# crabml/crabml

Hardware: NVIDIA H100
Metric: decode_tokens_per_s (higher is better)
Workload: dtype int8

## Files before the change

### crabml_b200/csrc/common.cuh

```cuda
#pragma once

#include <cuda_fp16.h>
#include <cuda_runtime.h>
#include <stdint.h>

#include <atomic>
#include <map>
#include <mutex>
#include <set>
#include <string>
#include <unordered_map>
#include <vector>

#include "../../include/crabml_cuda.h"

#define QK_K 256

#define CC_D_STRIDE(nb) ((((nb) + 7) / 8) * 8)
#define CC_HAS_PADDED_D(t) ((t) == CC_Q8_0 || (t) == CC_Q4_0)
#define CC_MAX_PLANES 4
#define CC_N_SLOTS 16
#define CC_HISTORY_CAP 65536

struct cc_device;
// ... 195 lines not shown
struct AttnArgs {
    const float *q, *k, *v;
    void *kcache, *vcache;
    float* out;
    void* act_scratch;
    const int64_t* dyn;
    const float* rope_tab;
    int n_heads, n_kv, hd, rope_dim, max_len, kv_f16;
    int64_t seq_stride;
    float scale;
};
struct DeqPlanes { const uint8_t* p[CC_MAX_PLANES]; int64_t cols; };
enum { MK_NORMQ = 0, MK_MATVEC = 1, MK_ATTN = 2, MK_ROWS = 3, MK_REDUCE = 4, MK_GATHER = 5, MK_ARGMAX = 6, MK_SAMPLE = 7 };
struct MkPhase {
    int type, wtype, write_back, next_matvec;
    int xgpu, red_n, spare1, spare; float* red_dst; const float* red_res;
    float* x; float* orig; const float* norm_w; float eps; int n; ActQ8_0 act;
    int act_type, spare2;
    StreamArgs mv;
    AttnArgs at;
    unsigned long long dyn_off, rope_off;
    DeqPlanes planes; int src_dtype, dst_dtype, n_rows, pad; long long cols; void* dst;
    const long long* rows_dev;
    long long* slot_dev; long long* hist_dev;
};
size_t cc_mega_smem_for_phase(const MkPhase& ph);
const CommDev* cc_comm_dev(cc_device* dev);
bool cc_comm_is_nccl(cc_device* dev);
int cc_comm_world(cc_device* dev);
void cc_comm_destroy(cc_device* dev);
int cc_launch_all_reduce(cc_device* dev, float* x, int64_t n, const float* residual);
int cc_launch_all_gather(cc_device* dev, const float* src, int64_t n, float* dst);
extern "C" CC_API int cc_test_mega_barrier_floor(cc_device* dev, int n, float* us_per_phase);
int cc_launch_mega(cc_device* dev, const MkPhase* phases_dev, int n_phases, const uint8_t* dyn_dev, unsigned* bar_dev, size_t smem_work, size_t smem_wstage,
                   unsigned long long* prof, bool sample);
bool cc_mega_test_stall();
bool cc_mega_ring_phase_ok(const MkPhase& ph);
int cc_mega_ring_at_ch(const MkPhase& ph);
size_t cc_mega_ring_smem_for_phase(const MkPhase& ph);
// ... 104 lines not shown
```

### crabml_b200/csrc/lazy.cu

```cuda
#include <math.h>
#include <stdlib.h>
#include <string.h>

#include <chrono>
#include <functional>

#include "sample_dev.cuh"

enum LKind { L_COPY_ROWS, L_DUP, L_RMS_NORM, L_MUL, L_ADD, L_SCALE, L_MATVEC, L_ROPE, L_CONCAT, L_CONTIGUOUS, L_BMM, L_SOFTMAX, L_SILU, L_GELU, L_ALLREDUCE, L_ALLGATHER, L_ARGMAX, L_SAMPLE };

struct LView { cc_buf* buf = nullptr; int ndim = 0; int64_t shape[CC_MAX_DIMS] = {0, 0, 0, 0}, strides[CC_MAX_DIMS] = {0, 0, 0, 0}; };

struct LOp {
    int kind;
    LView a, b;
    cc_buf* out = nullptr;
    float f = 0.0f;
    int64_t i0 = 0, i1 = 0, i2 = 0;
    std::vector<int64_t> rows;
    bool done = false;
};

struct GraphEntry { cudaGraphExec_t exec = nullptr; size_t dyn_bytes = 0; uint64_t launches = 0; MkPhase* phases_dev = nullptr;
                    std::vector<uint64_t> sig; uint64_t last_use = 0; int mega_variant = 0; };
// ... 38 lines not shown
static void graph_entry_free(GraphEntry& ge) {
    if (ge.exec) cudaGraphExecDestroy(ge.exec);
    if (ge.phases_dev) cudaFree(ge.phases_dev);
    ge.exec = nullptr; ge.phases_dev = nullptr;
}
static void graph_cache_clear(LazyState* lz) {
    for (auto& kv : lz->cache) graph_entry_free(kv.second);
    lz->cache.clear();
}

LazyState* cc_lazy_create(cc_device* dev) {
    LazyState* lz = new LazyState();
    for (int i = 0; i < LZ_DYN_SLOTS; i++)
        if (cudaMallocHost(&lz->dyn_host[i], lz->dyn_cap) != cudaSuccess || cudaEventCreateWithFlags(&lz->dyn_ev[i], cudaEventDisableTiming) != cudaSuccess) { delete lz; return nullptr; }
    if (cudaMalloc(&lz->dyn_dev, lz->dyn_cap) != cudaSuccess) { delete lz; return nullptr; }
    if (getenv("CRABML_MEGA_PROF")) cudaMalloc(&lz->prof_dev, 8 * 8 * 4097);
    if (cudaMalloc(&lz->bar_dev, 4096) != cudaSuccess || cudaMemset(lz->bar_dev, 0, 4096) != cudaSuccess) { delete lz; return nullptr; }
    return lz;
}
void cc_lazy_destroy(cc_device* dev) {
    LazyState* lz = dev->lz;
    if (!lz) return;
    for (auto& op : lz->q) { if (op.a.buf) cc_tensor_release(op.a.buf); if (op.b.buf) cc_tensor_release(op.b.buf); if (op.out) cc_tensor_release(op.out); }
    for (auto& kv : lz->cache) graph_entry_free(kv.second);
    lz->cache.clear();
    if (lz->bar_dev) cudaFree(lz->bar_dev);
    for (int i = 0; i < LZ_DYN_SLOTS; i++) { if (lz->dyn_host[i]) cudaFreeHost(lz->dyn_host[i]); if (lz->dyn_ev[i]) cudaEventDestroy(lz->dyn_ev[i]); }
    if (lz->dyn_dev) cudaFree(lz->dyn_dev);
    for (int i = 0; i < 2; i++) if (lz->act[i]) cudaFree(lz->act[i]);
    delete lz;
    dev->lz = nullptr;
// ... 47 lines not shown
    cc_device* dev;
    LazyState* lz;
    std::vector<LOp>& q;
    Plan& P;
    size_t rope_off = (size_t)-1; int64_t rope_pos = -1; int rope_hd = 0, rope_dim = 0;

    bool is(size_t i, int kind) const { return i < q.size() && !q[i].done && q[i].kind == kind; }
    std::unordered_map<cc_buf*, size_t> last_use;
    void index_uses() {
        last_use.reserve(q.size() * 2);
        for (size_t j = 0; j < q.size(); j++) {
            if (q[j].a.buf) last_use[q[j].a.buf] = j;
            if (q[j].b.buf) last_use[q[j].b.buf] = j;
            if (q[j].out) last_use[q[j].out] = j;
        }
    }
    bool dead_after(cc_buf* b, size_t from) const {
        auto lu = last_use.find(b);
        if (lu != last_use.end() && lu->second >= from) return false;
        auto it = lz->qrefs.find(b);
        int held = it == lz->qrefs.end() ? 0 : it->second;
        return b->refs.load() == held;
    }
    static bool same_dense_1xN(const LView& v, int64_t n) { return vcontig(v) && vlen(v) == n; }

    bool covered_by_phase = false;
    void fallback(size_t i) {
        if (!covered_by_phase) P.mega_ok = false;
        LOp op = q[i];
        cc_device* d = dev;
// ... 74 lines not shown
        if (rn.a.ndim > 2 || (rn.a.ndim == 2 && rn.a.shape[0] != 1) || !vcontig(rn.a) || n % 32) return 0;
        if (vlen(mu.b) != n || mu.b.buf->dtype != CC_F32 || !vcontig(mu.b)) return 0;
        if (n > 65536) return 0;
        float* x = (float*)rn.a.buf->plane[0];
        float* og = orig ? (float*)orig->base : nullptr;
        const float* w = (const float*)mu.b.buf->plane[0];
        float eps = rn.f;
        void* act = lz->act[act_sel];
        cc_device* d = dev;
        size_t end = j + 2;
        while (is(end, L_MATVEC) && q[end].b.buf == rn.a.buf && cc_stream_supported(q[end].a.buf->dtype, q[end].a.shape[1]) &&
               vlen(q[end].b) == q[end].a.shape[1] && vcontig(q[end].b)) end++;
        const bool write_back = !dead_after(rn.a.buf, end);
        P.S(0x2001); P.SP(x); P.SP(og); P.SP(w); P.SP(act); P.S((uint64_t)n); uint32_t eb; memcpy(&eb, &eps, 4); P.S(eb); P.S(write_back);
        P.steps.push_back([=](uint8_t*) { return cc_launch_normq(d, x, og, w, eps, n, act, write_back); });
        { MkPhase ph = {}; ph.type = MK_NORMQ; ph.write_back = write_back; ph.x = x; ph.orig = og; ph.norm_w = w; ph.eps = eps; ph.n = (int)n; ph.act = cc_act_q8_0(act, n); P.phases.push_back(ph); }
        *xbuf = rn.a.buf;
        size_t used = (j + 2) - i;
        for (size_t t = i; t < i + used; t++) q[t].done = true;
        return used;
    }

    size_t try_stream(size_t i, cc_buf* xbuf, int act_sel) {
        if (!is(i, L_MATVEC)) return 0;
        const LOp& m0 = q[i];
        const int wt = m0.a.buf->dtype;
        const int64_t k = m0.a.shape[1];
        if (!cc_stream_supported(wt, k) || m0.b.buf != xbuf || vlen(m0.b) != k || !vcontig(m0.b)) return 0;
        size_t n = 1;
        while (n < 3 && is(i + n, L_MATVEC) && q[i + n].b.buf == xbuf && q[i + n].a.buf->dtype == wt && q[i + n].a.shape[1] == k && vlen(q[i + n].b) == k) n++;
        StreamArgs A = {};
// ... 212 lines not shown
        } else if (n > 1 && is(j + n, L_SILU)) { n = 1; used_mv = 1; }
        if (is(j + used_mv, L_ALLREDUCE) || is(j + used_mv, L_ALLGATHER)) return 0;
        const size_t end = j + used_mv;
        if (norm_w && !dead_after(xb, end)) return 0;
        A.mats.n = (int)n;
        for (size_t t = 0; t < n; t++) {
            const cc_buf* w = q[j + t].a.buf;
            if (w->cols != k) return 0;
            A.mats.qs[t] = w->plane[0]; A.mats.d[t] = (const uint16_t*)w->plane[1]; A.mats.p2[t] = w->plane[2]; A.mats.p3[t] = w->plane[3];
            A.mats.out[t] = (float*)q[j + t].out->base;
            A.mats.m[t] = (int)q[j + t].a.shape[0];
        }
        MkPhase ph = {};
        ph.type = MK_MATVEC; ph.wtype = wt; ph.act_type = CC_Q8_K; ph.mv = A;
        ph.x = (float*)xb->plane[0]; ph.orig = orig ? (float*)orig->base : nullptr; ph.norm_w = norm_w; ph.eps = eps; ph.n = (int)k;
        covered_by_phase = true;
        for (size_t t = i; t < end; t++) fallback(t);
        covered_by_phase = false;
        P.phases.push_back(ph);
        P.mega_generic = true;
        return end - i;
    }

    void merge_prologue(size_t at) {
        const bool tail = at + 3 == P.phases.size() && (P.phases[at + 2].type == MK_REDUCE || P.phases[at + 2].type == MK_GATHER);
        if (at + 2 != P.phases.size() && !tail) return;
        MkPhase& nq = P.phases[at];
        MkPhase& mv = P.phases[at + 1];
        if (nq.type != MK_NORMQ || mv.type != MK_MATVEC || nq.write_back || nq.n != mv.mv.k) return;
        mv.x = nq.x; mv.orig = nq.orig; mv.norm_w = nq.norm_w; mv.eps = nq.eps; mv.n = nq.n;
        P.phases.erase(P.phases.begin() + at);
        if (at >= 1 && P.phases[at - 1].type == MK_REDUCE && P.phases[at - 1].red_dst == P.phases[at].x && P.phases[at - 1].red_n == P.phases[at].n) {
            MkPhase& m2 = P.phases[at];
            m2.red_n = P.phases[at - 1].red_n; m2.red_res = P.phases[at - 1].red_res;
            P.phases.erase(P.phases.begin() + (at - 1));
        }
    }

    void run() {
        index_uses();
        size_t i = 0;
        while (i < q.size()) {
            if (q[i].done) { i++; continue; }
            size_t used;
            cc_buf* xb = nullptr;
// ... 101 lines not shown
            if (use_mega && P.mega_sample) {
                int n_sample = 0;
                for (auto& ph : P.phases) n_sample += ph.type == MK_SAMPLE;
                if (n_sample != 1 || P.phases.back().type != MK_SAMPLE) use_mega = false;
            }
            if (use_mega) {
                bool stream = false, ring_ok = true;
                for (auto& ph : P.phases) {
                    if (ph.type == MK_MATVEC && ph.act_type != CC_Q8_K) stream = true;
                    if (!cc_mega_ring_phase_ok(ph)) ring_ok = false;
                }
                P.mega_ring = stream;
                for (auto& ph : P.phases) {
                    if (P.mega_ring) {
                        P.mega_smem = std::max(P.mega_smem, cc_mega_ring_smem_for_phase(ph));
                        if (ph.type == MK_MATVEC && ph.act_type == CC_Q8_K && ph.x && ph.norm_w) P.mega_wstage = std::max(P.mega_wstage, (size_t)ph.n * 4);
                        if (ph.type == MK_MATVEC && ph.act_type != CC_Q8_K) P.ring_slot = std::max(P.ring_slot, ph.wtype == CC_Q8_0 ? 4352 : 2304);
                        if (ph.type == MK_ATTN) P.ring_at_ch = cc_mega_ring_at_ch(ph);
                    } else {
                        P.mega_smem = std::max(P.mega_smem, cc_mega_smem_for_phase(ph));
                        if (ph.type == MK_MATVEC && ph.x && ph.norm_w) P.mega_wstage = std::max(P.mega_wstage, (size_t)ph.n * 4);
                    }
                }
                if (P.mega_ring) use_mega = ring_ok && cc_mega_ring_fits(P.mega_smem, P.mega_wstage, P.ring_slot, P.mega_generic);
                else use_mega = P.mega_smem + P.mega_wstage + 4096 <= 227 * 1024;
            }
            if (use_mega) {
                int nxt = -1;
                for (int t = (int)P.phases.size() - 1; t >= 0; t--) {
                    P.phases[t].next_matvec = nxt;
                    if (P.phases[t].type == MK_MATVEC) nxt = t;
                }
                if (cudaMalloc(&ge.phases_dev, P.phases.size() * sizeof(MkPhase)) != cudaSuccess ||
                    cudaMemcpy(ge.phases_dev, P.phases.data(), P.phases.size() * sizeof(MkPhase), cudaMemcpyHostToDevice) != cudaSuccess)
                    rc = cc_fail(dev, CC_ERR_CUDA, "lazy: phase table upload failed");
            }
            cudaError_t e = rc ? cudaSuccess : cudaStreamBeginCapture(dev->stream, cudaStreamCaptureModeRelaxed);
            if (!rc && e != cudaSuccess) rc = cc_fail(dev, CC_ERR_CUDA, "lazy: begin capture: %s", cudaGetErrorString(e));
            if (!rc) {
                if (use_mega && lz->prof_dev && P.phases.size() < 4000) { lz->prof_types.clear(); for (auto& ph : P.phases) lz->prof_types.push_back(ph.type * 16 + (ph.type == MK_MATVEC ? ph.mv.mats.n + 4 * ph.mv.epilogue + 1024 * (ph.mv.k >> 10) : 0)); }
                unsigned long long* prof = P.phases.size() < 4000 ? lz->prof_dev : nullptr;
                if (!use_mega) rc = run_steps(lz->dyn_dev);
                else if (P.mega_ring) rc = cc_launch_mega_ring(dev, ge.phases_dev, (int)P.phases.size(), lz->dyn_dev, lz->bar_dev, P.mega_smem, P.mega_wstage, prof, cc_comm_dev(dev),
                                                               P.mega_generic, P.mega_sample, P.ring_slot, P.ring_at_ch);
                else rc = cc_launch_mega(dev, ge.phases_dev, (int)P.phases.size(), lz->dyn_dev, lz->bar_dev, P.mega_smem, P.mega_wstage, prof, P.mega_sample);
                e = cudaStreamEndCapture(dev->stream, &graph);
// ... 39 lines not shown
int cc_check_async_error(cc_device* dev) {
    if (!dev || !dev->err_host) return CC_OK;
    const unsigned code = *(volatile unsigned*)dev->err_host;
    if (!code) return CC_OK;
    *(volatile unsigned*)dev->err_host = 0u;
    if (dev->err_dev) cudaMemset(dev->err_dev, 0, 256);
    if (dev->lz && dev->lz->bar_dev) cudaMemset(dev->lz->bar_dev, 0, 4096);
    return cc_fail(dev, CC_ERR_CUDA, "%s timeout (%s): the grid was not co-resident or a peer GPU stopped responding",
                   code == 3u ? "exchange kernel" : "megakernel barrier", code == 1u ? "grid barrier" : code == 4u ? "weight ring" : "cross-GPU handshake");
}

extern "C" CC_API int cc_lazy_mega_profile(cc_device* dev, unsigned long long* ts, int* types, int cap, int* n_out) {
    if (!dev || !dev->lz || !dev->lz->prof_dev || !ts || !types || !n_out) return CC_ERR_ARG;
    cudaStreamSynchronize(dev->stream);
    int n = (int)dev->lz->prof_types.size();
    if ((n + 1) * 8 > cap) return CC_ERR_ARG;
    if (cudaMemcpy(ts, dev->lz->prof_dev, (size_t)(n + 1) * 8 * 8, cudaMemcpyDeviceToHost) != cudaSuccess) return CC_ERR_CUDA;
    for (int i = 0; i < n; i++) types[i] = dev->lz->prof_types[i];
    *n_out = n;
    return CC_OK;
}

extern "C" CC_API int cc_lazy_mega_variant(cc_device* dev) { return dev && dev->lz ? dev->lz->mega_variant : 0; }

extern "C" CC_API int cc_lazy_stats(cc_device* dev, uint64_t* out4) {
    if (!dev || !dev->lz || !out4) return CC_ERR_ARG;
    out4[0] = dev->lz->flushes; out4[1] = dev->lz->graph_hits; out4[2] = dev->lz->captures; out4[3] = dev->lz->uncached;
    out4[4] = dev->lz->ns_record; out4[5] = dev->lz->ns_fuse; out4[6] = dev->lz->ns_submit; out4[7] = dev->lz->n_ops;
    return CC_OK;
}
```

### crabml_b200/csrc/mega_phases.cuh

```cuda
#pragma once
#include <stdlib.h>
#include <string.h>

#include "common.cuh"
#include "dequant.cuh"
#include "quantize_dev.cuh"
#include "vecdot.cuh"
#include "sample_dev.cuh"

#ifndef MK_SYNC
#error "define MK_SYNC() before including mega_phases.cuh"
#endif

#define MK_THREADS 512
#define MK_WARPS 16
#define MK_CTAS_PER_SM 1
#define MK_SEG 4
#define MK_XSTAGE_ROWS 512

__device__ __forceinline__ unsigned ld_acquire_u32(const unsigned* p) {
    unsigned v;
    asm volatile("ld.acquire.gpu.global.u32 %0, [%1];" : "=r"(v) : "l"(p) : "memory");
    return v;
}
// ... 460 lines not shown
        }
        return;
    }
    for (int i = blockIdx.x * MK_THREADS + threadIdx.x; i < n4; i += gridDim.x * MK_THREADS) {
        float4 a = __ldcg((const float4*)base + i);
        for (int p = 1; p < comm.world; p++) {
            const float4 b = __ldcg((const float4*)(base + (size_t)p * CC_COMM_MAX_ELEMS) + i);
            a.x += b.x; a.y += b.y; a.z += b.z; a.w += b.w;
        }
        if (ph.red_res) { const float4 r = __ldcg((const float4*)ph.red_res + i); a.x += r.x; a.y += r.y; a.z += r.z; a.w += r.w; }
        ((float4*)ph.red_dst)[i] = a;
    }
}


#define MK_PROF_SLOTS 8

#define MK_F_TESTSTALL 128
```

### crabml_b200/csrc/mega_ring.cu

```cuda
#define MK_SYNC() asm volatile("bar.sync 1, 512;" ::: "memory")
#define MK_GENERIC_NOINLINE 1
#include "mega_phases.cuh"

#define MR_PRODUCER_WARPS 4
#define MR_THREADS (MK_THREADS + 32 * MR_PRODUCER_WARPS)
#define MR_MAX_SLOTS 112
#define MR_Q8_SLOTS 24
#define MR_DESC_WORDS ((int)(sizeof(MkPhase) / 4))
#define MR_DESC_PER_LANE ((MR_DESC_WORDS + 31) / 32)

struct MrRing {
    int ring_off;
    int slot_bytes;
    int nslots;
    int at_ch;
};

__device__ __forceinline__ void mr_expect_tx(unsigned bar, unsigned bytes) { asm volatile("mbarrier.arrive.expect_tx.shared::cta.b64 _, [%0], %1;" ::"r"(bar), "r"(bytes) : "memory"); }
__device__ __forceinline__ void mr_bulk_g2s(unsigned dst, const void* src, unsigned bytes, unsigned bar) {
    asm volatile("cp.async.bulk.shared::cluster.global.mbarrier::complete_tx::bytes [%0], [%1], %2, [%3];" ::"r"(dst), "l"(src), "r"(bytes), "r"(bar) : "memory");
}
__device__ __forceinline__ bool mr_try_wait(unsigned bar, unsigned parity) {
    unsigned ok;
    asm volatile("{\n.reg .pred p;\nmbarrier.try_wait.parity.shared::cta.b64 p, [%1], %2;\nselp.u32 %0, 1, 0, p;\n}\n" : "=r"(ok) : "r"(bar), "r"(parity) : "memory");
    return ok != 0;
}
__device__ __forceinline__ void mr_release(unsigned done_addr, unsigned v, float dep) { asm volatile("st.release.cta.shared::cta.u32 [%0], %1;" ::"r"(done_addr), "r"(v), "f"(dep) : "memory"); }
__device__ __forceinline__ unsigned mr_ld_acquire_shared(unsigned addr) {
    unsigned v;
    asm volatile("ld.acquire.cta.shared::cta.u32 %0, [%1];" : "=r"(v) : "r"(addr) : "memory");
    return v;
}

struct MrGeo {
    int nb, GR, NSEG, V, E, n_units, first, stride, last_half_off, m_cat;
    bool pair;
// ... 18 lines not shown
    return g;
}
__device__ __forceinline__ int mr_locate(const StreamMats& M, const MrGeo& g, int rc, int v, int& mat) {
    mat = 0;
    int r = rc;
    if (g.pair) { mat = v; return r; }
    if (M.n > 1 && r >= M.m[0]) { r -= M.m[0]; mat = 1; if (M.n > 2 && r >= M.m[1]) { r -= M.m[1]; mat = 2; } }
    return r;
}

__device__ void mr_producer(const MkPhase* __restrict__ phases, int n_phases, const MrRing R, unsigned full0, unsigned done0, unsigned ring0,
                            MkPhase* s_pd, volatile unsigned* s_seq, volatile int* s_abort, int* s_prod_done, unsigned long long* prof_tail) {
    const int lane = threadIdx.x & 31;
    const int pt = (int)threadIdx.x - MK_THREADS;
    unsigned long long p_trips = 0, p_cyc = 0, p_iss = 0;
    for (int i = lane; i < MR_DESC_WORDS; i += 32) ((int*)&s_pd[0])[i] = ((const int*)phases)[i];
    __syncwarp();
    unsigned ent = 0;
    bool dead = false;
    for (int p = 0; p < n_phases && !dead; p++) {
        int nw[MR_DESC_PER_LANE];
#pragma unroll
        for (int j = 0; j < MR_DESC_PER_LANE; j++) { const int i = lane + 32 * j; nw[j] = (p + 1 < n_phases && i < MR_DESC_WORDS) ? ((const int*)(phases + p + 1))[i] : 0; }
        const MkPhase& ph = s_pd[p & 1];
        if (ph.type == MK_MATVEC && ph.act_type != CC_Q8_K) {
            const StreamArgs& A = ph.mv;
            const StreamMats& M = A.mats;
            const MrGeo g = mr_geo(A);
            const unsigned BB = ph.wtype == CC_Q8_0 ? 32u : 16u;
            const unsigned doff = MK_SEG * 32u * BB;
// ... 10 lines not shown
                    if (j < Npair) { const int P = j / twoE, w = j - P * twoE; u = 2 * P + (w & 1); vs = w >> 1; }
                    else { u = g.n_units - 1; vs = j - Npair; }
                    const int v = vs / g.NSEG, sg = vs - v * g.NSEG;
                    int mat;
                    const int r = mr_locate(M, g, g.first + u * g.stride, v, mat);
                    q0 = M.qs[mat] + ((size_t)r * g.nb + (size_t)sg * (MK_SEG * 32)) * BB;
                    d0 = M.d[mat] + (size_t)r * CC_D_STRIDE(g.nb) + sg * (MK_SEG * 32);
                    nbe = (unsigned)min(MK_SEG * 32, g.nb - MK_SEG * 32 * sg);
                    e = ent + (unsigned)j; slot = e % (unsigned)R.nslots; use = e / (unsigned)R.nslots;
                    have = true;
                }
                if (!use || mr_ld_acquire_shared(done0 + 4u * slot) == e - (unsigned)R.nslots + 1u) {
                    const unsigned fb = full0 + 8u * slot, dst = ring0 + slot * (unsigned)R.slot_bytes;
                    const unsigned dbytes = (nbe * 2u + 15u) & ~15u;
                    mr_expect_tx(fb, nbe * BB + dbytes);
                    mr_bulk_g2s(dst, q0, nbe * BB, fb);
                    mr_bulk_g2s(dst + doff, d0, dbytes, fb);
                    __threadfence_block();
                    s_seq[slot] = e + 1u;
                    j += 32 * MR_PRODUCER_WARPS; have = false; p_iss++;
                } else if ((++it & 0x3FFu) == 0 && *s_abort) { mydead = true; break; }
            }
            p_cyc += (unsigned long long)(clock64() - pc0);
            dead = __any_sync(0xffffffffu, mydead);
            ent += (unsigned)N;
        }
        __syncwarp();
#pragma unroll
        for (int j = 0; j < MR_DESC_PER_LANE; j++) { const int i = lane + 32 * j; if (i < MR_DESC_WORDS) ((int*)&s_pd[(p + 1) & 1])[i] = nw[j]; }
        __syncwarp();
    }
    if (lane == 0) { __threadfence_block(); atomicAdd(s_prod_done, 1); }
// ... 64 lines not shown
            const int asv = as_l[(seg * MK_SEG + g) * 32];
            const int4 loA = make_int4(wA.x & 0x0F0F0F0F, wA.y & 0x0F0F0F0F, wA.z & 0x0F0F0F0F, wA.w & 0x0F0F0F0F);
            const int4 hiA = make_int4((wA.x >> 4) & 0x0F0F0F0F, (wA.y >> 4) & 0x0F0F0F0F, (wA.z >> 4) & 0x0F0F0F0F, (wA.w >> 4) & 0x0F0F0F0F);
            const int4 loB = make_int4(wB.x & 0x0F0F0F0F, wB.y & 0x0F0F0F0F, wB.z & 0x0F0F0F0F, wB.w & 0x0F0F0F0F);
            const int4 hiB = make_int4((wB.x >> 4) & 0x0F0F0F0F, (wB.y >> 4) & 0x0F0F0F0F, (wB.z >> 4) & 0x0F0F0F0F, (wB.w >> 4) & 0x0F0F0F0F);
            const int sumA = mk_dp16(loA, alo) + mk_dp16(hiA, ahi) - 8 * asv;
            const int sumB = mk_dp16(loB, alo) + mk_dp16(hiB, ahi) - 8 * asv;
            accA += (float)sumA * h2f_bits(sA) * adv;
            accB += (float)sumB * h2f_bits(sB) * adv;
        }
    }
    partA = accA; partB = accB;
}

template <int TYPE>
__device__ void phase_matvec_ring(const MkPhase& ph, uint8_t* smem, const uint16_t* exp_lut, MrCons& RC, const CommDev& comm, unsigned xseq, unsigned long long* stamp1) {
    const StreamArgs& A = ph.mv;
    const int k = A.k;
    const MrGeo g = mr_geo(A);
    const int nb = g.nb, GR = g.GR, NSEG = g.NSEG;
    const bool pair = g.pair;
    const int nbp = NSEG * MK_SEG * 32;
    int8_t* s_q = (int8_t*)smem;
    float* s_d = (float*)(smem + (size_t)nbp * 32);
    int* s_s = (int*)(smem + (size_t)nbp * 32 + (size_t)nbp * 4);
    float* s_red = (float*)(smem + (size_t)nbp * 40);
    float* s_part = (float*)(smem + (size_t)nbp * 40 + 256);
    const int lane = threadIdx.x & 31, warp = threadIdx.x >> 5;
    const StreamMats& M = A.mats;
    if (threadIdx.x == 0) *RC.s_unit = 0;
    if (ph.x) {
        const int n4 = k >> 2;
        const int npass = nbp >> 6;
        const float4 z4 = make_float4(0, 0, 0, 0);
        const float* xbase = ph.red_n ? comm.data[comm.rank] + (size_t)(xseq & 1u) * CC_COMM_MAX_RANKS * CC_COMM_MAX_ELEMS : ph.x;
        auto load_x = [&](int i) -> float4 {
            if (i >= n4) return z4;
            float4 a4 = __ldcg((const float4*)xbase + i);
            if (ph.red_n) {
                for (int p = 1; p < comm.world; p++) {
                    const float4 t4 = __ldcg((const float4*)(xbase + (size_t)p * CC_COMM_MAX_ELEMS) + i);
                    a4.x += t4.x; a4.y += t4.y; a4.z += t4.z; a4.w += t4.w;
                }
                if (ph.red_res) { const float4 r4 = __ldcg((const float4*)ph.red_res + i); a4.x += r4.x; a4.y += r4.y; a4.z += r4.z; a4.w += r4.w; }
            }
            return a4;
        };
        float rms = 1.0f;
        const bool in_regs = npass <= 4;
        float4 xr[4], wr[4];
#pragma unroll
        for (int j = 0; j < 4; j++) { xr[j] = z4; wr[j] = z4; }
        if (in_regs) {
#pragma unroll
            for (int j = 0; j < 4; j++) {
                const int i = j * MK_THREADS + (int)threadIdx.x;
                if (j < npass) { xr[j] = load_x(i); if (ph.norm_w && i < n4) wr[j] = __ldg((const float4*)ph.norm_w + i); }
            }
        }
        if (stamp1) stamp1[3] = globaltimer_ns();
        if (ph.norm_w) {
            float ss = 0.0f;
            if (in_regs) {
#pragma unroll
                for (int j = 0; j < 4; j++) if (j * MK_THREADS + (int)threadIdx.x < n4) ss += cc_sq4(xr[j]);
            } else {
                for (int i = threadIdx.x; i < n4; i += MK_THREADS) { const float4 v = load_x(i); ss += cc_sq4(v); }
            }
            ss = warp_sum(ss);
            if (lane == 0) s_red[warp] = ss;
            MK_SYNC();
            float t = 0.0f;
#pragma unroll
            for (int w = 0; w < MK_WARPS; w++) t += s_red[w];
            rms = sqrtf(t / (float)k + ph.eps);
// ... 8 lines not shown
            float amax = fmaxf(fmaxf(fabsf(v.x), fabsf(v.y)), fmaxf(fabsf(v.z), fabsf(v.w)));
#pragma unroll
            for (int o = 4; o > 0; o >>= 1) amax = fmaxf(amax, __shfl_xor_sync(0xffffffffu, amax, o));
            const float d = amax / 127.0f;
            const int q0 = live ? __float2int_rz(v.x / d) : 0, q1 = live ? __float2int_rz(v.y / d) : 0;
            const int q2 = live ? __float2int_rz(v.z / d) : 0, q3 = live ? __float2int_rz(v.w / d) : 0;
            s_q32[mr_act_word(i)] = (q0 & 255) | ((q1 & 255) << 8) | ((q2 & 255) << 16) | (q3 << 24);
            if constexpr (TYPE == CC_Q4_0) {
                int sq = q0 + q1 + q2 + q3;
#pragma unroll
                for (int o = 4; o > 0; o >>= 1) sq += __shfl_xor_sync(0xffffffffu, sq, o);
                if (sub == 0) s_s[i >> 3] = sq;
            }
            if (sub == 0) s_d[i >> 3] = live ? __half2float(__float2half_rn(d)) : 0.0f;
        };
        if (in_regs) {
#pragma unroll
            for (int j = 0; j < 4; j++) if (j < npass) quant_chunk(j * MK_THREADS + (int)threadIdx.x, xr[j], wr[j]);
        } else {
            for (int j0 = 0; j0 < npass; j0 += 4) {
                float4 v[4], w4[4];
#pragma unroll
                for (int j = 0; j < 4; j++) {
                    const int i = (j0 + j) * MK_THREADS + (int)threadIdx.x;
                    v[j] = j0 + j < npass ? load_x(i) : z4;
                    w4[j] = (ph.norm_w && j0 + j < npass && i < n4) ? __ldg((const float4*)ph.norm_w + i) : z4;
                }
#pragma unroll
                for (int j = 0; j < 4; j++) if (j0 + j < npass) quant_chunk((j0 + j) * MK_THREADS + (int)threadIdx.x, v[j], w4[j]);
            }
        }
    } else {
        const uint8_t* act = (const uint8_t*)A.act;
        const int4* gq = (const int4*)act;
        int4* sq4 = (int4*)s_q;
        const float* gd = (const float*)(act + ((k + 15) & ~15));
        const int* gs = (const int*)(act + ((k + 15) & ~15) + ((nb * 4 + 15) & ~15));
        if (nbp <= MK_THREADS) {
            const int i0 = threadIdx.x, i1 = threadIdx.x + MK_THREADS;
            const int4 z4 = make_int4(0, 0, 0, 0);
            const int4 qa = i0 < nb * 2 ? __ldcg(gq + i0) : z4, qb = i1 < nb * 2 ? __ldcg(gq + i1) : z4;
            const float dv = i0 < nb ? __ldcg(gd + i0) : 0.0f;
            int sv = 0;
            if constexpr (TYPE == CC_Q4_0) sv = i0 < nb ? __ldcg(gs + i0) : 0;
            if (i0 < nbp * 2) sq4[mr_act_int4(i0)] = qa;
            if (i1 < nbp * 2) sq4[mr_act_int4(i1)] = qb;
            if (i0 < nbp) { s_d[i0] = dv; if constexpr (TYPE == CC_Q4_0) s_s[i0] = sv; }
        } else {
            for (int i = threadIdx.x; i < nbp * 2; i += MK_THREADS) sq4[mr_act_int4(i)] = i < nb * 2 ? __ldcg(gq + i) : make_int4(0, 0, 0, 0);
            for (int i = threadIdx.x; i < nbp; i += MK_THREADS) {
                s_d[i] = i < nb ? __ldcg(gd + i) : 0.0f;
                if constexpr (TYPE == CC_Q4_0) s_s[i] = i < nb ? __ldcg(gs + i) : 0;
            }
        }
    }
    MK_SYNC();
    if (stamp1) *stamp1 = globaltimer_ns();
    const int4* aq_l = (const int4*)s_q + lane;
    const float* ad_l = s_d + lane;
    const int* as_l = s_s + lane;
    float pend_a[2] = {0.0f, 0.0f}, pend_b[2] = {0.0f, 0.0f}, pend_res[2] = {0.0f, 0.0f};
    unsigned short pend_lut[2] = {0, 0};
    int pend_row[2] = {-1, -1};
    auto flush_pending = [&]() {
#pragma unroll
        for (int t = 0; t < 2; t++) {
            if (lane == 0 && pend_row[t] >= 0) {
                if (pair) M.out[0][pend_row[t]] = (pend_a[t] / (1.0f + h2f_bits(pend_lut[t]))) * pend_b[t];
                else M.out[0][pend_row[t]] = pend_a[t] + pend_res[t];
            }
            pend_row[t] = -1;
        }
// ... 92 lines not shown
        for (int i = 0; i < R.nslots; i++) { mbar_init(full0 + 8u * i, 1u); s_done[i] = 0u; s_seq[i] = 0u; }
        s_abort = 0; s_prod_done = 0; s_ring_dead = 0;
    }
    asm volatile("fence.mbarrier_init.release.cluster;" ::: "memory");
    asm volatile("fence.proxy.async.shared::cta;" ::: "memory");
    __syncthreads();
    if (threadIdx.x >= MK_THREADS) {
        mr_producer(phases, n_phases, R, full0, done0, (unsigned)__cvta_generic_to_shared(smem + R.ring_off), s_pd[(threadIdx.x - MK_THREADS) >> 5], s_seq, &s_abort, &s_prod_done,
                    prof ? prof + (size_t)n_phases * MK_PROF_SLOTS : nullptr);
        return;
    }
    MrCons RC;
    RC.full0 = full0; RC.done0 = done0; RC.ring = smem + R.ring_off; RC.slot_bytes = R.slot_bytes; RC.nslots = R.nslots; RC.ent_base = 0u;
    RC.s_unit = &s_unit; RC.s_seq = s_seq; RC.s_dead = &s_ring_dead; RC.err_dev = &bar[MK_BAR_ERR]; RC.err_host = err_host;
    uint8_t* work = smem;
    float* s_w = (float*)(smem + wtop_off);
    unsigned gen = 0;
    if (threadIdx.x == MK_BAR_THREAD) gen = ld_acquire_u32(&bar[32]);
    unsigned xseq = comm.world > 0 ? *comm.seq : 0u;
    for (int i = threadIdx.x; i < MR_DESC_WORDS; i += MK_THREADS) ((int*)&s_phs[0])[i] = ((const int*)phases)[i];
    const int n_loop = SMP ? n_phases - 1 : n_phases;
    for (int p = 0; p < n_loop; p++) {
        const bool stamp = prof && blockIdx.x == 0 && threadIdx.x == 0;
        if (stamp) { prof[p * MK_PROF_SLOTS] = globaltimer_ns(); prof[p * MK_PROF_SLOTS + 1] = 0; prof[p * MK_PROF_SLOTS + 4] = 0; prof[p * MK_PROF_SLOTS + 5] = 0; }
        MK_SYNC();
        const MkPhase& s_ph = s_phs[p & 1];
        static_assert(sizeof(MkPhase) / 4 <= MK_THREADS, "descriptor does not fit one word per thread");
        int desc_w = 0;
        if (p + 1 < n_phases && threadIdx.x < sizeof(MkPhase) / 4) desc_w = ((const int*)(phases + p + 1))[threadIdx.x];
        unsigned long long* st1 = stamp ? prof + p * MK_PROF_SLOTS + 1 : nullptr;
        switch (s_ph.type) {
        case MK_NORMQ: phase_normq(s_ph, s_red); break;
        case MK_MATVEC:
            if (GEN && s_ph.act_type == CC_Q8_K) {
                switch (s_ph.wtype) {
                case CC_Q2_K: phase_matvec_generic<TQ2_K>(s_ph, work, s_w, false, false, exp_lut, st1); break;
                case CC_Q3_K: phase_matvec_generic<TQ3_K>(s_ph, work, s_w, false, false, exp_lut, st1); break;
                case CC_Q4_K: phase_matvec_generic<TQ45_K<false>>(s_ph, work, s_w, false, false, exp_lut, st1); break;
                case CC_Q5_K: phase_matvec_generic<TQ45_K<true>>(s_ph, work, s_w, false, false, exp_lut, st1); break;
                case CC_Q6_K: phase_matvec_generic<TQ6_K>(s_ph, work, s_w, false, false, exp_lut, st1); break;
                default: phase_matvec_generic<TQ8_K>(s_ph, work, s_w, false, false, exp_lut, st1); break;
                }
                break;
            }
            if (s_ph.wtype == CC_Q8_0) phase_matvec_ring<CC_Q8_0>(s_ph, work, exp_lut, RC, comm, xseq, st1);
            else phase_matvec_ring<CC_Q4_0>(s_ph, work, exp_lut, RC, comm, xseq, st1);
            break;
        case MK_ATTN:
            if (s_ph.at.kv_f16) phase_attn<true>(s_ph, (float*)work, s_red, dyn, exp_lut, abar0, apar, R.at_ch);
            else phase_attn<false>(s_ph, (float*)work, s_red, dyn, exp_lut, abar0, apar, R.at_ch);
            break;
        case MK_ROWS: phase_rows(s_ph, dyn); break;
        case MK_REDUCE: phase_reduce(s_ph, comm, xseq, false); break;
        case MK_GATHER: phase_reduce(s_ph, comm, xseq, true); break;
        case MK_ARGMAX: phase_argmax(s_ph, dyn, s_red); break;
        }
        if (stamp) prof[p * MK_PROF_SLOTS + 2] = globaltimer_ns();
        if (p + 1 < n_phases && threadIdx.x < sizeof(MkPhase) / 4) ((int*)&s_phs[(p + 1) & 1])[threadIdx.x] = desc_w;
        const bool more = p + 1 < n_phases;
        const bool xg = s_ph.xgpu != 0;
        if (test_stall && p == 2 && blockIdx.x == gridDim.x - 1) { if (threadIdx.x == 0) s_abort = 1; break; }
        if (more) grid_barrier_arrive(bar, gridDim.x, gen);
        if (stamp) prof[p * MK_PROF_SLOTS + 3] = globaltimer_ns();
        if (more) {
            grid_barrier_wait(bar, gridDim.x, gen, comm, xg ? xseq + 1u : 0u, &s_abort, err_host);
            gen++; if (xg) xseq++;
            if (s_abort) break;
        }
    }
    if constexpr (SMP) {
        MK_SYNC();
        if (!s_abort) phase_sample(s_phs[(n_phases - 1) & 1], dyn, work, exp_lut);
    }
    if (comm.world > 0 && blockIdx.x == 0 && threadIdx.x == 0) *comm.seq = xseq;
    if (prof && blockIdx.x == 0 && threadIdx.x == 0) prof[n_phases * MK_PROF_SLOTS] = globaltimer_ns();
    MK_SYNC();
    if (s_abort && threadIdx.x == 0) {
        while (*(volatile int*)&s_prod_done < MR_PRODUCER_WARPS) {}
        for (unsigned sl = 0; sl < (unsigned)R.nslots; sl++) {
            const unsigned q = *(volatile unsigned*)&s_seq[sl];
            if (q) mbar_wait(full0 + 8u * sl, ((q - 1u) / (unsigned)R.nslots) & 1u);
        }
    }
}

bool cc_mega_ring_phase_ok(const MkPhase& ph) {
    if (ph.type != MK_MATVEC || ph.act_type == CC_Q8_K) return true;
    if (ph.wtype != CC_Q8_0 && ph.wtype != CC_Q4_0) return false;
    if (ph.mv.k % 32) return false;
    for (int t = 0; t < ph.mv.mats.n; t++)
        if (((uintptr_t)ph.mv.mats.qs[t] | (uintptr_t)ph.mv.mats.d[t]) & 15u) return false;
    return true;
}
int cc_mega_ring_at_ch(const MkPhase& ph) {
    return ph.at.kv_f16 ? 64 : 32;
}
size_t cc_mega_ring_smem_for_phase(const MkPhase& ph) {
    if (ph.type == MK_MATVEC && ph.act_type == CC_Q8_K) return cc_mega_smem_for_phase(ph);
    if (ph.type == MK_MATVEC) {
        const size_t k = (size_t)ph.mv.k, nb = k / 32, GR = (nb + 31) / 32, NSEG = (GR + MK_SEG - 1) / MK_SEG, nbp = NSEG * MK_SEG * 32;
        return nbp * 40 + 256 + 2048;
    }
    if (ph.type == MK_ATTN) return (size_t)(3 * ph.at.hd + ((ph.at.max_len + 8 + 3) & ~3)) * 4 + (size_t)AT_NBUF * cc_mega_ring_at_ch(ph) * ph.at.hd * (ph.at.kv_f16 ? 2 : 4) + 64;
    if (ph.type == MK_SAMPLE) return SMP_SMEM_BYTES;
    return 1024;
}
#define MR_MIN_SLOTS 12
static size_t mr_ring_off(size_t smem_work, size_t smem_wstage) { return ((((smem_work + 15) & ~(size_t)15) + smem_wstage) + 127) & ~(size_t)127; }
int cc_mega_ring_slots(size_t smem_work, size_t smem_wstage, int slot_bytes, bool generic) {
    cudaFuncAttributes fa;
    if (cudaFuncGetAttributes(&fa, generic ? mega_ring_kernel<true, false> : mega_ring_kernel<false, false>) != cudaSuccess) { cudaGetLastError(); return 0; }
    const size_t cap = 227 * 1024 - fa.sharedSizeBytes, off = mr_ring_off(smem_work, smem_wstage);
    if (slot_bytes <= 0 || off >= cap) return 0;
    const size_t n = (cap - off) / (size_t)slot_bytes;
    return (int)(n > MR_MAX_SLOTS ? MR_MAX_SLOTS : n);
}
bool cc_mega_ring_fits(size_t smem_work, size_t smem_wstage, int slot_bytes, bool generic) { return cc_mega_ring_slots(smem_work, smem_wstage, slot_bytes, generic) >= MR_MIN_SLOTS; }
// ... 35 lines not shown
```

Baseline: 266.8.

## Prefetch next RMSNorm weights and activations into shared memory across phases

Uses cp.async to stage the next fused norm+matvec phase's RMSNorm weights into shared memory during the preceding matvec. The input activation vector is likewise staged right after the grid barrier, instead of being loaded from global memory inside the quantize step. It also adds an L2 evict_first cache hint to the bulk weight-streaming copies so streamed weights do not displace reusable data in L2. The aim is to hide the latency of these global loads behind other work. The cost is a larger shared-memory footprint per phase, which may reduce the ring slot count, plus extra profiling slots and planner metadata.

```diff
diff --git a/crabml_b200/csrc/common.cuh b/crabml_b200/csrc/common.cuh
--- a/crabml_b200/csrc/common.cuh
+++ b/crabml_b200/csrc/common.cuh
@@ -233,15 +233,16 @@
 enum { MK_NORMQ = 0, MK_MATVEC = 1, MK_ATTN = 2, MK_ROWS = 3, MK_REDUCE = 4, MK_GATHER = 5, MK_ARGMAX = 6, MK_SAMPLE = 7 };
 struct MkPhase {
     int type, wtype, write_back, next_matvec;
-    int xgpu, red_n, spare1, spare; float* red_dst; const float* red_res;
+    int xgpu, red_n; const float* next_norm_w; float* red_dst; const float* red_res;
     float* x; float* orig; const float* norm_w; float eps; int n; ActQ8_0 act;
-    int act_type, spare2;
+    int act_type, next_norm_n;
     StreamArgs mv;
     AttnArgs at;
     unsigned long long dyn_off, rope_off;
     DeqPlanes planes; int src_dtype, dst_dtype, n_rows, pad; long long cols; void* dst;
     const long long* rows_dev;
     long long* slot_dev; long long* hist_dev;
+    int norm_ahead, pad2;
 };
 size_t cc_mega_smem_for_phase(const MkPhase& ph);
 const CommDev* cc_comm_dev(cc_device* dev);
diff --git a/crabml_b200/csrc/lazy.cu b/crabml_b200/csrc/lazy.cu
--- a/crabml_b200/csrc/lazy.cu
+++ b/crabml_b200/csrc/lazy.cu
@@ -76,7 +76,7 @@
     for (int i = 0; i < LZ_DYN_SLOTS; i++)
         if (cudaMallocHost(&lz->dyn_host[i], lz->dyn_cap) != cudaSuccess || cudaEventCreateWithFlags(&lz->dyn_ev[i], cudaEventDisableTiming) != cudaSuccess) { delete lz; return nullptr; }
     if (cudaMalloc(&lz->dyn_dev, lz->dyn_cap) != cudaSuccess) { delete lz; return nullptr; }
-    if (getenv("CRABML_MEGA_PROF")) cudaMalloc(&lz->prof_dev, 8 * 8 * 4097);
+    if (getenv("CRABML_MEGA_PROF") && cudaMalloc(&lz->prof_dev, 9 * 8 * 4097) == cudaSuccess) cudaMemset(lz->prof_dev, 0, 9 * 8 * 4097);
     if (cudaMalloc(&lz->bar_dev, 4096) != cudaSuccess || cudaMemset(lz->bar_dev, 0, 4096) != cudaSuccess) { delete lz; return nullptr; }
     return lz;
 }
@@ -154,6 +154,10 @@
             if (q[j].b.buf) last_use[q[j].b.buf] = j;
             if (q[j].out) last_use[q[j].out] = j;
         }
+    }
+    bool written(const cc_buf* b) const {
+        for (const LOp& op : q) if (op.a.buf == b || op.out == b) return true;
+        return false;
     }
     bool dead_after(cc_buf* b, size_t from) const {
         auto lu = last_use.find(b);
@@ -258,7 +262,8 @@
         const bool write_back = !dead_after(rn.a.buf, end);
         P.S(0x2001); P.SP(x); P.SP(og); P.SP(w); P.SP(act); P.S((uint64_t)n); uint32_t eb; memcpy(&eb, &eps, 4); P.S(eb); P.S(write_back);
         P.steps.push_back([=](uint8_t*) { return cc_launch_normq(d, x, og, w, eps, n, act, write_back); });
-        { MkPhase ph = {}; ph.type = MK_NORMQ; ph.write_back = write_back; ph.x = x; ph.orig = og; ph.norm_w = w; ph.eps = eps; ph.n = (int)n; ph.act = cc_act_q8_0(act, n); P.phases.push_back(ph); }
+        { MkPhase ph = {}; ph.type = MK_NORMQ; ph.write_back = write_back; ph.x = x; ph.orig = og; ph.norm_w = w; ph.eps = eps; ph.n = (int)n; ph.act = cc_act_q8_0(act, n);
+          ph.norm_ahead = !written(mu.b.buf); P.phases.push_back(ph); }
         *xbuf = rn.a.buf;
         size_t used = (j + 2) - i;
         for (size_t t = i; t < i + used; t++) q[t].done = true;
@@ -501,6 +506,7 @@
         MkPhase ph = {};
         ph.type = MK_MATVEC; ph.wtype = wt; ph.act_type = CC_Q8_K; ph.mv = A;
         ph.x = (float*)xb->plane[0]; ph.orig = orig ? (float*)orig->base : nullptr; ph.norm_w = norm_w; ph.eps = eps; ph.n = (int)k;
+        ph.norm_ahead = norm_w && !written(q[j - 1].b.buf);
         covered_by_phase = true;
         for (size_t t = i; t < end; t++) fallback(t);
         covered_by_phase = false;
@@ -515,7 +521,7 @@
         MkPhase& nq = P.phases[at];
         MkPhase& mv = P.phases[at + 1];
         if (nq.type != MK_NORMQ || mv.type != MK_MATVEC || nq.write_back || nq.n != mv.mv.k) return;
-        mv.x = nq.x; mv.orig = nq.orig; mv.norm_w = nq.norm_w; mv.eps = nq.eps; mv.n = nq.n;
+        mv.x = nq.x; mv.orig = nq.orig; mv.norm_w = nq.norm_w; mv.eps = nq.eps; mv.n = nq.n; mv.norm_ahead = nq.norm_ahead;
         P.phases.erase(P.phases.begin() + at);
         if (at >= 1 && P.phases[at - 1].type == MK_REDUCE && P.phases[at - 1].red_dst == P.phases[at].x && P.phases[at - 1].red_n == P.phases[at].n) {
             MkPhase& m2 = P.phases[at];
@@ -647,7 +653,7 @@
                 for (auto& ph : P.phases) {
                     if (P.mega_ring) {
                         P.mega_smem = std::max(P.mega_smem, cc_mega_ring_smem_for_phase(ph));
-                        if (ph.type == MK_MATVEC && ph.act_type == CC_Q8_K && ph.x && ph.norm_w) P.mega_wstage = std::max(P.mega_wstage, (size_t)ph.n * 4);
+                        if (ph.type == MK_MATVEC && ph.x && ph.norm_w) P.mega_wstage = std::max(P.mega_wstage, (size_t)ph.n * 4);
                         if (ph.type == MK_MATVEC && ph.act_type != CC_Q8_K) P.ring_slot = std::max(P.ring_slot, ph.wtype == CC_Q8_0 ? 4352 : 2304);
                         if (ph.type == MK_ATTN) P.ring_at_ch = cc_mega_ring_at_ch(ph);
                     } else {
@@ -659,10 +665,14 @@
                 else use_mega = P.mega_smem + P.mega_wstage + 4096 <= 227 * 1024;
             }
             if (use_mega) {
-                int nxt = -1;
+                int nxt = -1, nxn = -1;
                 for (int t = (int)P.phases.size() - 1; t >= 0; t--) {
-                    P.phases[t].next_matvec = nxt;
-                    if (P.phases[t].type == MK_MATVEC) nxt = t;
+                    MkPhase& ph = P.phases[t];
+                    ph.next_matvec = nxt;
+                    ph.next_norm_w = nxn >= 0 && P.phases[nxn].norm_ahead ? P.phases[nxn].norm_w : nullptr;
+                    ph.next_norm_n = ph.next_norm_w ? P.phases[nxn].n : 0;
+                    if (ph.type == MK_MATVEC) nxt = t;
+                    if (ph.type == MK_MATVEC && ph.x && ph.norm_w) nxn = t;
                 }
                 if (cudaMalloc(&ge.phases_dev, P.phases.size() * sizeof(MkPhase)) != cudaSuccess ||
                     cudaMemcpy(ge.phases_dev, P.phases.data(), P.phases.size() * sizeof(MkPhase), cudaMemcpyHostToDevice) != cudaSuccess)
@@ -732,8 +742,8 @@
     if (!dev || !dev->lz || !dev->lz->prof_dev || !ts || !types || !n_out) return CC_ERR_ARG;
     cudaStreamSynchronize(dev->stream);
     int n = (int)dev->lz->prof_types.size();
-    if ((n + 1) * 8 > cap) return CC_ERR_ARG;
-    if (cudaMemcpy(ts, dev->lz->prof_dev, (size_t)(n + 1) * 8 * 8, cudaMemcpyDeviceToHost) != cudaSuccess) return CC_ERR_CUDA;
+    if ((n + 1) * 9 > cap) return CC_ERR_ARG;
+    if (cudaMemcpy(ts, dev->lz->prof_dev, (size_t)(n + 1) * 9 * 8, cudaMemcpyDeviceToHost) != cudaSuccess) return CC_ERR_CUDA;
     for (int i = 0; i < n; i++) types[i] = dev->lz->prof_types[i];
     *n_out = n;
     return CC_OK;
diff --git a/crabml_b200/csrc/mega_phases.cuh b/crabml_b200/csrc/mega_phases.cuh
--- a/crabml_b200/csrc/mega_phases.cuh
+++ b/crabml_b200/csrc/mega_phases.cuh
@@ -498,6 +498,6 @@
 }
 
 
-#define MK_PROF_SLOTS 8
+#define MK_PROF_SLOTS 9
 
 #define MK_F_TESTSTALL 128
diff --git a/crabml_b200/csrc/mega_ring.cu b/crabml_b200/csrc/mega_ring.cu
--- a/crabml_b200/csrc/mega_ring.cu
+++ b/crabml_b200/csrc/mega_ring.cu
@@ -17,9 +17,16 @@
 };
 
 __device__ __forceinline__ void mr_expect_tx(unsigned bar, unsigned bytes) { asm volatile("mbarrier.arrive.expect_tx.shared::cta.b64 _, [%0], %1;" ::"r"(bar), "r"(bytes) : "memory"); }
-__device__ __forceinline__ void mr_bulk_g2s(unsigned dst, const void* src, unsigned bytes, unsigned bar) {
-    asm volatile("cp.async.bulk.shared::cluster.global.mbarrier::complete_tx::bytes [%0], [%1], %2, [%3];" ::"r"(dst), "l"(src), "r"(bytes), "r"(bar) : "memory");
-}
+__device__ __forceinline__ void mr_bulk_g2s(unsigned dst, const void* src, unsigned bytes, unsigned bar, unsigned long long pol) {
+    asm volatile("cp.async.bulk.shared::cluster.global.mbarrier::complete_tx::bytes.L2::cache_hint [%0], [%1], %2, [%3], %4;" ::"r"(dst), "l"(src), "r"(bytes), "r"(bar), "l"(pol) : "memory");
+}
+__device__ __forceinline__ void mr_stage_f32(float* dst, const float* src, int n) {
+    const unsigned s = (unsigned)__cvta_generic_to_shared(dst);
+    for (int i = threadIdx.x; i < (n >> 2); i += MK_THREADS) asm volatile("cp.async.cg.shared.global [%0], [%1], 16;" ::"r"(s + i * 16), "l"(src + i * 4) : "memory");
+    asm volatile("cp.async.commit_group;" ::: "memory");
+}
+__host__ __device__ __forceinline__ int mr_nbp(int k) { const int GR = ((k >> 5) + 31) >> 5; return (GR + MK_SEG - 1) / MK_SEG * MK_SEG * 32; }
+__host__ __device__ __forceinline__ int mr_x_off(int k) { return mr_nbp(k) * 40 + 256 + 2048; }
 __device__ __forceinline__ bool mr_try_wait(unsigned bar, unsigned parity) {
     unsigned ok;
     asm volatile("{\n.reg .pred p;\nmbarrier.try_wait.parity.shared::cta.b64 p, [%1], %2;\nselp.u32 %0, 1, 0, p;\n}\n" : "=r"(ok) : "r"(bar), "r"(parity) : "memory");
@@ -68,6 +75,8 @@
     const int lane = threadIdx.x & 31;
     const int pt = (int)threadIdx.x - MK_THREADS;
     unsigned long long p_trips = 0, p_cyc = 0, p_iss = 0;
+    unsigned long long pol;
+    asm volatile("createpolicy.fractional.L2::evict_first.b64 %0, 1.0;" : "=l"(pol));
     for (int i = lane; i < MR_DESC_WORDS; i += 32) ((int*)&s_pd[0])[i] = ((const int*)phases)[i];
     __syncwarp();
     unsigned ent = 0;
@@ -108,8 +117,8 @@
                     const unsigned fb = full0 + 8u * slot, dst = ring0 + slot * (unsigned)R.slot_bytes;
                     const unsigned dbytes = (nbe * 2u + 15u) & ~15u;
                     mr_expect_tx(fb, nbe * BB + dbytes);
-                    mr_bulk_g2s(dst, q0, nbe * BB, fb);
-                    mr_bulk_g2s(dst + doff, d0, dbytes, fb);
+                    mr_bulk_g2s(dst, q0, nbe * BB, fb, pol);
+                    mr_bulk_g2s(dst + doff, d0, dbytes, fb, pol);
                     __threadfence_block();
                     s_seq[slot] = e + 1u;
                     j += 32 * MR_PRODUCER_WARPS; have = false; p_iss++;
@@ -204,7 +213,8 @@
 }
 
 template <int TYPE>
-__device__ void phase_matvec_ring(const MkPhase& ph, uint8_t* smem, const uint16_t* exp_lut, MrCons& RC, const CommDev& comm, unsigned xseq, unsigned long long* stamp1) {
+__device__ void phase_matvec_ring(const MkPhase& ph, uint8_t* smem, float* s_wn, const float*& wst, bool x_staged, const uint16_t* exp_lut, MrCons& RC,
+                                  const CommDev& comm, unsigned xseq, unsigned long long* stamp1) {
     const StreamArgs& A = ph.mv;
     const int k = A.k;
     const MrGeo g = mr_geo(A);
@@ -223,32 +233,35 @@
         const int n4 = k >> 2;
         const int npass = nbp >> 6;
         const float4 z4 = make_float4(0, 0, 0, 0);
+        const float4* s_w4 = (const float4*)s_wn;
+        const float4* s_x4 = (const float4*)(smem + mr_x_off(k));
         const float* xbase = ph.red_n ? comm.data[comm.rank] + (size_t)(xseq & 1u) * CC_COMM_MAX_RANKS * CC_COMM_MAX_ELEMS : ph.x;
         auto load_x = [&](int i) -> float4 {
             if (i >= n4) return z4;
+            if (!ph.red_n) return s_x4[i];
             float4 a4 = __ldcg((const float4*)xbase + i);
-            if (ph.red_n) {
-                for (int p = 1; p < comm.world; p++) {
-                    const float4 t4 = __ldcg((const float4*)(xbase + (size_t)p * CC_COMM_MAX_ELEMS) + i);
-                    a4.x += t4.x; a4.y += t4.y; a4.z += t4.z; a4.w += t4.w;
-                }
-                if (ph.red_res) { const float4 r4 = __ldcg((const float4*)ph.red_res + i); a4.x += r4.x; a4.y += r4.y; a4.z += r4.z; a4.w += r4.w; }
-            }
+            for (int p = 1; p < comm.world; p++) {
+                const float4 t4 = __ldcg((const float4*)(xbase + (size_t)p * CC_COMM_MAX_ELEMS) + i);
+                a4.x += t4.x; a4.y += t4.y; a4.z += t4.z; a4.w += t4.w;
+            }
+            if (ph.red_res) { const float4 r4 = __ldcg((const float4*)ph.red_res + i); a4.x += r4.x; a4.y += r4.y; a4.z += r4.z; a4.w += r4.w; }
             return a4;
         };
+        if (ph.norm_w && ph.norm_w != wst) { mr_stage_f32(s_wn, ph.norm_w, k); wst = ph.norm_w; }
+        if (!ph.red_n && !x_staged) mr_stage_f32((float*)s_x4, ph.x, k);
+        asm volatile("cp.async.wait_group 1;" ::: "memory");
+        if (stamp1) stamp1[7] = globaltimer_ns();
+        asm volatile("cp.async.wait_group 0;" ::: "memory");
+        if (stamp1) stamp1[3] = globaltimer_ns();
         float rms = 1.0f;
-        const bool in_regs = npass <= 4;
-        float4 xr[4], wr[4];
-#pragma unroll
-        for (int j = 0; j < 4; j++) { xr[j] = z4; wr[j] = z4; }
+        const bool in_regs = ph.red_n && npass <= 4;
+        float4 xr[4];
+#pragma unroll
+        for (int j = 0; j < 4; j++) xr[j] = z4;
         if (in_regs) {
 #pragma unroll
-            for (int j = 0; j < 4; j++) {
-                const int i = j * MK_THREADS + (int)threadIdx.x;
-                if (j < npass) { xr[j] = load_x(i); if (ph.norm_w && i < n4) wr[j] = __ldg((const float4*)ph.norm_w + i); }
-            }
-        }
-        if (stamp1) stamp1[3] = globaltimer_ns();
+            for (int j = 0; j < 4; j++) if (j < npass) xr[j] = load_x(j * MK_THREADS + (int)threadIdx.x);
+        }
         if (ph.norm_w) {
             float ss = 0.0f;
             if (in_regs) {
@@ -287,20 +300,19 @@
             }
             if (sub == 0) s_d[i >> 3] = live ? __half2float(__float2half_rn(d)) : 0.0f;
         };
+        auto load_w = [&](int i) -> float4 { return ph.norm_w && i < n4 ? s_w4[i] : z4; };
         if (in_regs) {
 #pragma unroll
-            for (int j = 0; j < 4; j++) if (j < npass) quant_chunk(j * MK_THREADS + (int)threadIdx.x, xr[j], wr[j]);
+            for (int j = 0; j < 4; j++) if (j < npass) quant_chunk(j * MK_THREADS + (int)threadIdx.x, xr[j], load_w(j * MK_THREADS + (int)threadIdx.x));
+        } else if (!ph.red_n) {
+            for (int j = 0; j < npass; j++) { const int i = j * MK_THREADS + (int)threadIdx.x; quant_chunk(i, load_x(i), load_w(i)); }
         } else {
             for (int j0 = 0; j0 < npass; j0 += 4) {
-                float4 v[4], w4[4];
-#pragma unroll
-                for (int j = 0; j < 4; j++) {
-                    const int i = (j0 + j) * MK_THREADS + (int)threadIdx.x;
-                    v[j] = j0 + j < npass ? load_x(i) : z4;
-                    w4[j] = (ph.norm_w && j0 + j < npass && i < n4) ? __ldg((const float4*)ph.norm_w + i) : z4;
-                }
-#pragma unroll
-                for (int j = 0; j < 4; j++) if (j0 + j < npass) quant_chunk((j0 + j) * MK_THREADS + (int)threadIdx.x, v[j], w4[j]);
+                float4 v[4];
+#pragma unroll
+                for (int j = 0; j < 4; j++) v[j] = j0 + j < npass ? load_x((j0 + j) * MK_THREADS + (int)threadIdx.x) : z4;
+#pragma unroll
+                for (int j = 0; j < 4; j++) if (j0 + j < npass) quant_chunk((j0 + j) * MK_THREADS + (int)threadIdx.x, v[j], load_w((j0 + j) * MK_THREADS + (int)threadIdx.x));
             }
         }
     } else {
@@ -329,6 +341,7 @@
     }
     MK_SYNC();
     if (stamp1) *stamp1 = globaltimer_ns();
+    if (ph.x && ph.norm_w) { wst = ph.next_norm_w; if (wst) mr_stage_f32(s_wn, wst, ph.next_norm_n); }
     const int4* aq_l = (const int4*)s_q + lane;
     const float* ad_l = s_d + lane;
     const int* as_l = s_s + lane;
@@ -451,7 +464,9 @@
     RC.full0 = full0; RC.done0 = done0; RC.ring = smem + R.ring_off; RC.slot_bytes = R.slot_bytes; RC.nslots = R.nslots; RC.ent_base = 0u;
     RC.s_unit = &s_unit; RC.s_seq = s_seq; RC.s_dead = &s_ring_dead; RC.err_dev = &bar[MK_BAR_ERR]; RC.err_host = err_host;
     uint8_t* work = smem;
-    float* s_w = (float*)(smem + wtop_off);
+    float* s_wn = (float*)(smem + wtop_off);
+    const float* wst = nullptr;
+    int xstaged = -1;
     unsigned gen = 0;
     if (threadIdx.x == MK_BAR_THREAD) gen = ld_acquire_u32(&bar[32]);
     unsigned xseq = comm.world > 0 ? *comm.seq : 0u;
@@ -459,9 +474,10 @@
     const int n_loop = SMP ? n_phases - 1 : n_phases;
     for (int p = 0; p < n_loop; p++) {
         const bool stamp = prof && blockIdx.x == 0 && threadIdx.x == 0;
-        if (stamp) { prof[p * MK_PROF_SLOTS] = globaltimer_ns(); prof[p * MK_PROF_SLOTS + 1] = 0; prof[p * MK_PROF_SLOTS + 4] = 0; prof[p * MK_PROF_SLOTS + 5] = 0; }
+        if (stamp) { prof[p * MK_PROF_SLOTS] = globaltimer_ns(); prof[p * MK_PROF_SLOTS + 1] = 0; prof[p * MK_PROF_SLOTS + 4] = 0; prof[p * MK_PROF_SLOTS + 5] = 0; prof[p * MK_PROF_SLOTS + 8] = 0; }
         MK_SYNC();
         const MkPhase& s_ph = s_phs[p & 1];
+        if (p == 0 && !(s_ph.type == MK_MATVEC && s_ph.x && s_ph.norm_w)) { wst = s_ph.next_norm_w; if (wst) mr_stage_f32(s_wn, wst, s_ph.next_norm_n); }
         static_assert(sizeof(MkPhase) / 4 <= MK_THREADS, "descriptor does not fit one word per thread");
         int desc_w = 0;
         if (p + 1 < n_phases && threadIdx.x < sizeof(MkPhase) / 4) desc_w = ((const int*)(phases + p + 1))[threadIdx.x];
@@ -471,17 +487,18 @@
         case MK_MATVEC:
             if (GEN && s_ph.act_type == CC_Q8_K) {
                 switch (s_ph.wtype) {
-                case CC_Q2_K: phase_matvec_generic<TQ2_K>(s_ph, work, s_w, false, false, exp_lut, st1); break;
-                case CC_Q3_K: phase_matvec_generic<TQ3_K>(s_ph, work, s_w, false, false, exp_lut, st1); break;
-                case CC_Q4_K: phase_matvec_generic<TQ45_K<false>>(s_ph, work, s_w, false, false, exp_lut, st1); break;
-                case CC_Q5_K: phase_matvec_generic<TQ45_K<true>>(s_ph, work, s_w, false, false, exp_lut, st1); break;
-                case CC_Q6_K: phase_matvec_generic<TQ6_K>(s_ph, work, s_w, false, false, exp_lut, st1); break;
-                default: phase_matvec_generic<TQ8_K>(s_ph, work, s_w, false, false, exp_lut, st1); break;
+                case CC_Q2_K: phase_matvec_generic<TQ2_K>(s_ph, work, s_wn, s_ph.norm_w == wst, false, exp_lut, st1); break;
+                case CC_Q3_K: phase_matvec_generic<TQ3_K>(s_ph, work, s_wn, s_ph.norm_w == wst, false, exp_lut, st1); break;
+                case CC_Q4_K: phase_matvec_generic<TQ45_K<false>>(s_ph, work, s_wn, s_ph.norm_w == wst, false, exp_lut, st1); break;
+                case CC_Q5_K: phase_matvec_generic<TQ45_K<true>>(s_ph, work, s_wn, s_ph.norm_w == wst, false, exp_lut, st1); break;
+                case CC_Q6_K: phase_matvec_generic<TQ6_K>(s_ph, work, s_wn, s_ph.norm_w == wst, false, exp_lut, st1); break;
+                default: phase_matvec_generic<TQ8_K>(s_ph, work, s_wn, s_ph.norm_w == wst, false, exp_lut, st1); break;
                 }
+                if (s_ph.x && s_ph.norm_w) { wst = s_ph.next_norm_w; if (wst) mr_stage_f32(s_wn, wst, s_ph.next_norm_n); }
                 break;
             }
-            if (s_ph.wtype == CC_Q8_0) phase_matvec_ring<CC_Q8_0>(s_ph, work, exp_lut, RC, comm, xseq, st1);
-            else phase_matvec_ring<CC_Q4_0>(s_ph, work, exp_lut, RC, comm, xseq, st1);
+            if (s_ph.wtype == CC_Q8_0) phase_matvec_ring<CC_Q8_0>(s_ph, work, s_wn, wst, xstaged == p, exp_lut, RC, comm, xseq, st1);
+            else phase_matvec_ring<CC_Q4_0>(s_ph, work, s_wn, wst, xstaged == p, exp_lut, RC, comm, xseq, st1);
             break;
         case MK_ATTN:
             if (s_ph.at.kv_f16) phase_attn<true>(s_ph, (float*)work, s_red, dyn, exp_lut, abar0, apar, R.at_ch);
@@ -503,8 +520,11 @@
             grid_barrier_wait(bar, gridDim.x, gen, comm, xg ? xseq + 1u : 0u, &s_abort, err_host);
             gen++; if (xg) xseq++;
             if (s_abort) break;
-        }
-    }
+            const MkPhase& nph = s_phs[(p + 1) & 1];
+            if (nph.type == MK_MATVEC && nph.act_type != CC_Q8_K && nph.x && !nph.red_n) { mr_stage_f32((float*)(work + mr_x_off(nph.mv.k)), nph.x, nph.mv.k); xstaged = p + 1; }
+        }
+    }
+    asm volatile("cp.async.wait_all;" ::: "memory");
     if constexpr (SMP) {
         MK_SYNC();
         if (!s_abort) phase_sample(s_phs[(n_phases - 1) & 1], dyn, work, exp_lut);
@@ -534,10 +554,7 @@
 }
 size_t cc_mega_ring_smem_for_phase(const MkPhase& ph) {
     if (ph.type == MK_MATVEC && ph.act_type == CC_Q8_K) return cc_mega_smem_for_phase(ph);
-    if (ph.type == MK_MATVEC) {
-        const size_t k = (size_t)ph.mv.k, nb = k / 32, GR = (nb + 31) / 32, NSEG = (GR + MK_SEG - 1) / MK_SEG, nbp = NSEG * MK_SEG * 32;
-        return nbp * 40 + 256 + 2048;
-    }
+    if (ph.type == MK_MATVEC) return (size_t)mr_x_off(ph.mv.k) + (ph.x && !ph.red_n ? (size_t)ph.mv.k * 4 : 0);
     if (ph.type == MK_ATTN) return (size_t)(3 * ph.at.hd + ((ph.at.max_len + 8 + 3) & ~3)) * 4 + (size_t)AT_NBUF * cc_mega_ring_at_ch(ph) * ph.at.hd * (ph.at.kv_f16 ? 2 : 4) + 64;
     if (ph.type == MK_SAMPLE) return SMP_SMEM_BYTES;
     return 1024;
```

Result: faster. 277.1, median of 6 (+3.9%).
